# kakao/buffalo

Hardware: NVIDIA H100
Metric: interactions/sec (nnz/s) ALS d=128 (higher is better)
Workload: dtype f32

## Files before the change

buffalo_b200/csrc/als_tc.cuh:

```cuda
#pragma once
#include "als_generic.cuh"
#include "bfl_common.cuh"
#include <type_traits>

#include "sm90_ptx.cuh"

namespace bfl {
namespace tc {

using namespace sm90;

constexpr int N_CONV = 4, KH = N_CONV / 4;
constexpr int W_EPI = 0, W_MMA = 4, W_CONV = 8, W_PLAN = W_CONV + N_CONV;
constexpr int WARPS = 16, THREADS = WARPS * 32;
constexpr int REG_MMA = 200, REG_PLAN = 4 * 128 - 128 - 128 - REG_MMA;
constexpr int NXS = 8;
constexpr int PT = 2;
constexpr int NR = 2;
constexpr int NO = 2;
constexpr int GATHER_AHEAD = 1;
constexpr int NPG = 8, NP = NPG * PT;
constexpr int NBV = 8;
template <int D>
struct Cfg {
    static constexpr int TILE = D == 128 ? 32 : 16;
    static constexpr int NF = D / 128;
    static constexpr int LBO = D * 16;
    static constexpr int OP_BYTES = TILE * D * 2;
};
constexpr uint32_t F_FIRST = 1u << 8, F_LAST = 1u << 9, F_NEG = 1u << 10, F_STOP = 1u << 11;

__device__ __forceinline__ int msw(int c) { return ((c >> 1) & 3) << 3; }

template <int D>
struct Smem {
    static constexpr int TILE = Cfg<D>::TILE;
    alignas(1024) unsigned char op[NO][PT][2][Cfg<D>::OP_BYTES];
    alignas(128) float raw[NR][PT][TILE * D];
    alignas(128) float mat[128 * 128];
    alignas(16) float bvec[NBV][KH][D];
    alignas(16) float sumq[NBV][KH][D];
    alignas(16) float xs[NXS][D];
    alignas(16) float pv[4][32];
    alignas(16) float dl[4][32];
    alignas(16) float sws[NP][TILE];
    alignas(16) float wv[NP][TILE];
    alignas(16) int32_t keys[NP][TILE];
    float wsum[NBV][KH];
    uint32_t meta_raw[NP];
    uint32_t meta_op[NO][PT];
    int badrow[NXS];
    alignas(8) uint64_t plan_full[NPG], plan_empty[NPG], raw_full[NR], raw_empty[NR], op_full[NO], op_empty[NO];
    alignas(8) uint64_t acc_full, acc_empty, x_full[NXS], d_full[4];
};

struct TcArgs {
    AlsArgs a;
    const int32_t* items;
    float* scratch;
    int64_t split;
    int pass;
    int debug;
};

template <int D>
__host__ __device__ constexpr size_t scratch_floats() { return (size_t)D * D + 2 * D + 4; }

__global__ void tc_absmax_kernel(const float* __restrict__ p, size_t n, unsigned int* __restrict__ out) {
    float m = 0.f;
    const size_t gtid = (size_t)blockIdx.x * blockDim.x + threadIdx.x, gsz = (size_t)gridDim.x * blockDim.x;
    const size_t lead = min(n, (size_t)(((16 - ((uintptr_t)p & 15)) & 15) / 4));
    const size_t n4 = (n - lead) / 4;
    const float4* p4 = reinterpret_cast<const float4*>(p + lead);
    for (size_t i = gtid; i < n4; i += gsz) {
        const float4 v = __ldg(p4 + i);
        m = fmaxf(fmaxf(m, fmaxf(fabsf(v.x), fabsf(v.y))), fmaxf(fabsf(v.z), fabsf(v.w)));
    }
    for (size_t i = gtid; i < lead; i += gsz) m = fmaxf(m, fabsf(p[i]));
    for (size_t i = lead + n4 * 4 + gtid; i < n; i += gsz) m = fmaxf(m, fabsf(p[i]));
    for (int o = 16; o > 0; o >>= 1) m = fmaxf(m, __shfl_xor_sync(FULL, m, o));
    if ((threadIdx.x & 31) == 0 && m > 0.f) atomicMax(out, __float_as_uint(m));
}
__global__ void tc_scale_kernel(const unsigned int* __restrict__ ymax, const unsigned int* __restrict__ vmax, float alpha,
                                float* __restrict__ out) {
    const float y = __uint_as_float(*ymax), w = __uint_as_float(*vmax) * fabsf(alpha);
    const float top = y * sqrtf(w);
    int e = 0;
    if (top > 0.f && isfinite(top)) {
        int ex;
        frexpf(top, &ex);
        e = 15 - ex;
    }
    e = max(-60, min(60, e));
    out[0] = ldexpf(1.f, e);
    out[1] = ldexpf(1.f, -2 * e);
}

template <int D, bool PARTIAL, bool LOSS1>
__global__ void __launch_bounds__(THREADS, 1) als_tc_kernel(TcArgs ta) {
    static_assert(D == 128 || (D == 256 && PARTIAL), "fused row solve: d = 128; split-row mode: d = 128 or 256");
    constexpr int TILE = Cfg<D>::TILE, NF = Cfg<D>::NF, LBO = Cfg<D>::LBO;
    extern __shared__ __align__(1024) unsigned char smem_raw_[];
    Smem<D>& S = *reinterpret_cast<Smem<D>*>(smem_raw_);
    const AlsArgs& a = ta.a;
    const int tid = threadIdx.x, lane = tid & 31;
    const int warp = __shfl_sync(FULL, tid >> 5, 0);

    if (tid == 0) {
        for (int i = 0; i < NR; ++i) {
            mbar_init(&S.raw_full[i], N_CONV);
            mbar_init(&S.raw_empty[i], N_CONV);
        }
        for (int i = 0; i < NPG; ++i) {
            mbar_init(&S.plan_full[i], 1);
            mbar_init(&S.plan_empty[i], N_CONV);
        }
        for (int i = 0; i < NO; ++i) {
            mbar_init(&S.op_full[i], N_CONV);
            mbar_init(&S.op_empty[i], 4);
        }
        mbar_init(&S.acc_full, 4);
        mbar_init(&S.acc_empty, 4);
        for (int b = 0; b < 4; ++b) mbar_init(&S.d_full[b], 1);
        for (int i = 0; i < NXS; ++i) {
            mbar_init(&S.x_full[i], 4);
            S.badrow[i] = 0;
        }
        mbar_init_fence();
    }
    __syncthreads();
    const float scale = __ldg(a.tc_scales), inv2 = __ldg(a.tc_scales + 1);

    const int64_t nitems = a.row_end - a.row_begin;
    const int64_t my_first = (int64_t)blockIdx.x;
    const int64_t stride = gridDim.x;

    auto item_info = [&](int64_t it, int& row, int64_t& beg, int64_t& n, int& slot) {
        if (PARTIAL) {
            const int32_t* p = ta.items + 3 * (a.row_begin + it);
            row = p[0];
            const int64_t rb = row == 0 ? 0 : a.indptr[row - 1];
            const int64_t rn = a.indptr[row] - rb;
            beg = rb + (int64_t)p[1] * ta.split;
            n = min(ta.split, rn - (int64_t)p[1] * ta.split);
            slot = p[2];
        } else {
            row = a.row_list[a.row_begin + it];
            beg = row == 0 ? 0 : a.indptr[row - 1];
            n = a.indptr[row] - beg;
            slot = 0;
        }
    };

    if (warp >= W_PLAN) {
        setmaxnreg_dec<REG_PLAN>();
        if (warp != W_PLAN) return;
        uint32_t gsl = 0, rph = 0, pe = 0;
        auto tile_begin = [&]() -> uint32_t {
            if (pe == 0) mbar_wait_idle(&S.plan_empty[gsl], rph ^ 1u);
            return gsl * PT + pe;
        };
        auto tile_end = [&]() {
            if (++pe == PT) {
                if (lane == 0) mbar_arrive(&S.plan_full[gsl]);
                pe = 0;
                if (++gsl == NPG) { gsl = 0; rph ^= 1u; }
            }
        };
        auto emit = [&](unsigned mask, uint32_t flags, int32_t key, float w) {
            const int cnt = __popc(mask);
            const int slot = __popc(mask & ((1u << lane) - 1u));
            const uint32_t rs = tile_begin();
            if ((mask >> lane) & 1u) {
                S.keys[rs][slot] = key;
                S.sws[rs][slot] = sqrtf(fabsf(w)) * scale;
                S.wv[rs][slot] = w;
            } else {
                const int zslot = cnt + lane - slot;
                if (zslot < TILE) {
                    S.sws[rs][zslot] = 0.f;
                    S.wv[rs][zslot] = 0.f;
                }
            }
            if (lane == 0) S.meta_raw[rs] = (uint32_t)cnt | flags;
            __syncwarp();
            tile_end();
        };
        constexpr int SC = 4, SCN = SC * TILE;
        const bool inl = lane < TILE;
        auto load_id = [&](int64_t it, int& row, int& chunk) {
            row = -1;
            chunk = 0;
            if (it < nitems) {
                if (PARTIAL) {
                    const int32_t* p = ta.items + 3 * (a.row_begin + it);
                    row = p[0];
                    chunk = p[1];
                } else {
                    row = a.row_list[a.row_begin + it];
                }
            }
        };
        auto load_span = [&](int row, int chunk, const int32_t*& kp, const float*& vp, int& n) {
            kp = a.keys;
            vp = a.vals;
            n = 0;
            if (row >= 0) {
                const int64_t rb = row == 0 ? 0 : a.indptr[row - 1];
                const int64_t rn = a.indptr[row] - rb;
                int64_t beg = rb;
                n = (int)rn;
                if (PARTIAL) {
                    beg = rb + (int64_t)chunk * ta.split;
                    n = (int)min(ta.split, rn - (int64_t)chunk * ta.split);
                }
                kp = a.keys + (beg - a.shift);
                vp = a.vals + (beg - a.shift);
            }
        };
        auto load_sc = [&](const int32_t* kp, const float* vp, int n, int c0, int32_t (&key)[SC], float (&w)[SC]) {
#pragma unroll
            for (int s = 0; s < SC; ++s) {
                const int idx = c0 + s * TILE + lane;
                const bool ok = inl && idx < n;
                key[s] = ok ? kp[idx] : 0;
                w[s] = ok ? vp[idx] * a.alpha : 0.f;
            }
        };
        auto emit_sc = [&](int n, int c0, const int32_t (&key)[SC], const float (&w)[SC]) {
            bool neg = false;
#pragma unroll
            for (int s = 0; s < SC; ++s) neg |= w[s] < 0.f;
            if (!__any_sync(FULL, neg)) {
#pragma unroll
                for (int s = 0; s < SC; ++s) {
                    const int t0 = c0 + s * TILE;
                    if (t0 < n) {
                        const uint32_t meta = (uint32_t)min(TILE, n - t0) | (t0 == 0 ? F_FIRST : 0u) | (t0 + TILE >= n ? F_LAST : 0u);
                        const uint32_t rs = tile_begin();
                        if (inl) {
                            float sq;
                            asm("sqrt.approx.ftz.f32 %0, %1;" : "=f"(sq) : "f"(w[s]));
                            S.keys[rs][lane] = key[s];
                            S.sws[rs][lane] = sq * scale;
                            S.wv[rs][lane] = w[s];
                        }
                        if (lane == 0) S.meta_raw[rs] = meta;
                        __syncwarp();
                        tile_end();
                    }
                }
            } else {
#pragma unroll
                for (int s = 0; s < SC; ++s) {
                    const int t0 = c0 + s * TILE;
                    if (t0 < n) {
                        const bool valid = inl && t0 + lane < n;
                        const unsigned pm = __ballot_sync(FULL, valid && !(w[s] < 0.f));
                        const unsigned nm = __ballot_sync(FULL, valid && (w[s] < 0.f));
                        const bool lastc = t0 + TILE >= n;
                        uint32_t fl = (t0 == 0 ? F_FIRST : 0u);
                        if (pm) {
                            emit(pm, fl | ((lastc && !nm) ? F_LAST : 0u), key[s], w[s]);
                            fl = 0u;
                        }
                        if (nm) emit(nm, fl | F_NEG | (lastc ? F_LAST : 0u), key[s], w[s]);
                    }
                }
            }
        };
        const int32_t *kp0, *kp1, *kp2, *kp3;
        const float *vp0, *vp1, *vp2, *vp3;
        int n0, n1, n2, n3;
        int row_t, ch_t, row4, ch4;
        int32_t k0[SC], k1[SC], k2[SC], nk[SC];
        float w0[SC], w1[SC], w2[SC], nw[SC];
        load_id(my_first, row_t, ch_t);
        load_span(row_t, ch_t, kp0, vp0, n0);
        load_sc(kp0, vp0, n0, 0, k0, w0);
        load_id(my_first + stride, row_t, ch_t);
        load_span(row_t, ch_t, kp1, vp1, n1);
        load_sc(kp1, vp1, n1, 0, k1, w1);
        load_id(my_first + 2 * stride, row_t, ch_t);
        load_span(row_t, ch_t, kp2, vp2, n2);
        load_id(my_first + 3 * stride, row4, ch4);
        for (int64_t it = my_first; it < nitems; it += stride) {
            load_sc(kp2, vp2, n2, 0, k2, w2);
            load_span(row4, ch4, kp3, vp3, n3);
            load_id(it + 4 * stride, row4, ch4);
            for (int c0 = 0; c0 < n0; c0 += SCN) {
                const bool more = c0 + SCN < n0;
                if (more) load_sc(kp0, vp0, n0, c0 + SCN, nk, nw);
                emit_sc(n0, c0, k0, w0);
                if (more) {
#pragma unroll
                    for (int s = 0; s < SC; ++s) { k0[s] = nk[s]; w0[s] = nw[s]; }
                }
            }
#pragma unroll
            for (int s = 0; s < SC; ++s) { k0[s] = k1[s]; w0[s] = w1[s]; k1[s] = k2[s]; w1[s] = w2[s]; }
            kp0 = kp1; vp0 = vp1; n0 = n1; kp1 = kp2; vp1 = vp2; n1 = n2; kp2 = kp3; vp2 = vp3; n2 = n3;
        }
        do {
            const uint32_t rs = tile_begin();
            if (lane == 0) S.meta_raw[rs] = F_STOP;
            __syncwarp();
            tile_end();
        } while (pe != 0);
    } else if (warp >= W_MMA && warp < W_MMA + 4) {
        setmaxnreg_inc<REG_MMA>();
        const int r0 = (D == 256 && ta.pass == 2) ? 128 : 0, c0 = (D == 256 && ta.pass > 0) ? 128 : 0;
        const int wq = warp - W_MMA;
        const int fr = 16 * wq + (lane >> 2), fc = 2 * (lane & 3);
        float d0[64], d1[64];
        auto acc_init = [&]() {
            const float s2 = scale * scale;
#pragma unroll
            for (int n = 0; n < 16; ++n)
#pragma unroll
                for (int h = 0; h < 2; ++h) {
                    const int r = fr + 8 * h, c = 8 * n + fc;
                    float2 g0 = make_float2(0.f, 0.f), g1 = make_float2(0.f, 0.f);
                    if (!PARTIAL) {
                        g0 = __ldg(reinterpret_cast<const float2*>(a.G + (size_t)r * D + c));
                        g1 = __ldg(reinterpret_cast<const float2*>(a.G + (size_t)(r + 64) * D + c));
                        g0.x += r == c ? a.reg : 0.f;
                        g0.y += r == c + 1 ? a.reg : 0.f;
                        g1.x += r + 64 == c ? a.reg : 0.f;
                        g1.y += r + 64 == c + 1 ? a.reg : 0.f;
                    }
                    d0[4 * n + 2 * h] = g0.x * s2; d0[4 * n + 2 * h + 1] = g0.y * s2;
                    d1[4 * n + 2 * h] = g1.x * s2; d1[4 * n + 2 * h + 1] = g1.y * s2;
                }
        };
        uint32_t os = 0, oph = 0, aph = 0;
        int64_t seq = 0;
        bool stop = false;
        acc_init();
        while (!stop) {
            mbar_wait(&S.op_full[os], oph);
            fence_proxy_async_smem();
#pragma unroll 1
            for (int e = 0; e < PT; ++e) {
                const uint32_t meta = S.meta_op[os][e];
                if (meta & F_STOP) {
                    stop = true;
                    break;
                }
                const int ksteps = (ta.debug & 2) ? 0 : (int)(meta & 0xffu);
                const uint32_t hi = s32(&S.op[os][e][0][0]), lo = s32(&S.op[os][e][1][0]);
                wgmma_fence();
#pragma unroll 1
                for (int ks = 0; ks < ksteps; ++ks) {
                    const uint32_t k0 = ks * 2 * LBO;
                    const uint64_t ah0 = smem_desc(hi + k0 + r0 * 16, LBO, 128), ah1 = smem_desc(hi + k0 + (r0 + 64) * 16, LBO, 128);
                    const uint64_t al0 = smem_desc(lo + k0 + r0 * 16, LBO, 128), al1 = smem_desc(lo + k0 + (r0 + 64) * 16, LBO, 128);
                    const uint64_t bh = smem_desc(hi + k0 + c0 * 16, LBO, 128), bl = smem_desc(lo + k0 + c0 * 16, LBO, 128);
                    if (meta & F_NEG) {
                        wgmma_m64n128k16_f16<true>(d0, ah0, bh);
                        wgmma_m64n128k16_f16<true>(d0, ah0, bl);
                        wgmma_m64n128k16_f16<true>(d0, al0, bh);
                        wgmma_m64n128k16_f16<true>(d1, ah1, bh);
                        wgmma_m64n128k16_f16<true>(d1, ah1, bl);
                        wgmma_m64n128k16_f16<true>(d1, al1, bh);
                    } else {
                        wgmma_m64n128k16_f16<false>(d0, ah0, bh);
                        wgmma_m64n128k16_f16<false>(d0, ah0, bl);
                        wgmma_m64n128k16_f16<false>(d0, al0, bh);
                        wgmma_m64n128k16_f16<false>(d1, ah1, bh);
                        wgmma_m64n128k16_f16<false>(d1, ah1, bl);
                        wgmma_m64n128k16_f16<false>(d1, al1, bh);
                    }
                }
                wgmma_commit();
                if (meta & F_LAST) {
                    wgmma_wait<0>();
#pragma unroll
                    for (int i = 0; i < 64; ++i) { acc_fence(d0[i]); acc_fence(d1[i]); }
                    mbar_wait_idle(&S.acc_empty, aph ^ 1u);
                    if (PARTIAL) {
                        const int slot = ta.items[3 * (a.row_begin + my_first + seq * stride) + 2];
                        float* sc = ta.scratch + (size_t)slot * scratch_floats<D>();
#pragma unroll
                        for (int n = 0; n < 16; ++n)
#pragma unroll
                            for (int h = 0; h < 2; ++h)
#pragma unroll
                                for (int i = 0; i < 2; ++i) {
                                    const int r = r0 + fr + 8 * h, c = c0 + 8 * n + fc + i;
                                    const float v0 = d0[4 * n + 2 * h + i] * inv2, v1 = d1[4 * n + 2 * h + i] * inv2;
                                    atomicAdd(sc + (size_t)r * D + c, v0);
                                    atomicAdd(sc + (size_t)(r + 64) * D + c, v1);
                                    if (r0 != c0) {
                                        atomicAdd(sc + (size_t)c * D + r, v0);
                                        atomicAdd(sc + (size_t)c * D + r + 64, v1);
                                    }
                                }
                    } else {
#pragma unroll
                        for (int n = 0; n < 16; ++n)
#pragma unroll
                            for (int h = 0; h < 2; ++h)
#pragma unroll
                                for (int i = 0; i < 2; ++i) {
                                    const int r = fr + 8 * h, c = 8 * n + fc + i;
                                    S.mat[c * 128 + (r ^ msw(c))] = d0[4 * n + 2 * h + i] * inv2;
                                    S.mat[c * 128 + ((r + 64) ^ msw(c))] = d1[4 * n + 2 * h + i] * inv2;
                                }
                    }
                    __syncwarp();
                    if (lane == 0) mbar_arrive(&S.acc_full);
                    aph ^= 1u;
                    ++seq;
                    acc_init();
                }
            }
            wgmma_wait<0>();
#pragma unroll
            for (int i = 0; i < 64; ++i) { acc_fence(d0[i]); acc_fence(d1[i]); }
            __syncwarp();
            if (lane == 0) mbar_arrive(&S.op_empty[os]);
            if (++os == NO) { os = 0; oph ^= 1u; }
        }
    } else if (warp >= W_CONV && warp < W_CONV + N_CONV) {
        const int cta = tid - W_CONV * 32;
        const int ct = cta & 127;
        const int kh = cta >> 7;
        constexpr int CHS = TILE / 8 / KH;
        uint32_t rs = 0, rph = 0, os = 0, oph = 0, bslot = 0;
        float2 bacc[NF], qacc[NF];
        float wacc = 0.f;
#pragma unroll
        for (int f = 0; f < NF; ++f) { bacc[f] = make_float2(0.f, 0.f); qacc[f] = make_float2(0.f, 0.f); }
        const int cw = cta >> 5;
        uint32_t gs = 0, gph = 0, grs = 0, grph = 0;
        bool plan_end = false;
        auto gather = [&]() {
            if (plan_end) {
                cp_async_commit();
                return;
            }
            mbar_wait(&S.plan_full[gs], gph);
            mbar_wait(&S.raw_empty[grs], grph ^ 1u);
            const uint32_t gm0 = S.meta_raw[gs * PT], gm1 = S.meta_raw[gs * PT + 1];
            if (PT == 2 && !(ta.debug & 1) && ((gm0 | gm1) & F_STOP) == 0 && (gm0 & 0xffu) == TILE && (gm1 & 0xffu) == TILE) {
                int32_t kk[PT][TILE / N_CONV];
#pragma unroll
                for (int e = 0; e < PT; ++e)
#pragma unroll
                    for (int i = 0; i < TILE / N_CONV; ++i) kk[e][i] = S.keys[gs * PT + e][cw + N_CONV * i];
#pragma unroll
                for (int e = 0; e < PT; ++e)
#pragma unroll
                    for (int i = 0; i < TILE / N_CONV; ++i) {
                        const float* src = a.Y + (int64_t)kk[e][i] * a.ld + lane * 4;
                        float* dst = &S.raw[grs][e][(cw + N_CONV * i) * D + lane * 4];
#pragma unroll
                        for (int c = 0; c < D / 128; ++c) cp_async16_cg(dst + c * 128, src + c * 128);
                    }
            } else
#pragma unroll
            for (int e = 0; e < PT; ++e) {
                const uint32_t gmeta = S.meta_raw[gs * PT + e];
                if (gmeta & F_STOP) {
                    plan_end = true;
                } else {
                    const int gcnt = (ta.debug & 1) ? 0 : (int)(gmeta & 0xffu);
#pragma unroll
                    for (int i = 0; i < TILE / N_CONV; ++i) {
                        const int slot = cw + N_CONV * i;
                        if (slot < gcnt) {
                            const float* src = a.Y + (int64_t)S.keys[gs * PT + e][slot] * a.ld + lane * 4;
                            float* dst = &S.raw[grs][e][slot * D + lane * 4];
#pragma unroll
                            for (int c = 0; c < D / 128; ++c) cp_async16_cg(dst + c * 128, src + c * 128);
                        }
                    }
                }
            }
            cp_async_commit();
            if (++gs == NPG) { gs = 0; gph ^= 1u; }
            if (++grs == NR) { grs = 0; grph ^= 1u; }
        };
        uint32_t cs = 0;
        bool done = false;
        if (ta.debug & 16) {
            uint32_t ph = 0;
            for (;;) {
                mbar_wait(&S.plan_full[cs], ph);
                const bool stop = (S.meta_raw[cs * PT] | S.meta_raw[cs * PT + 1]) & F_STOP;
                __syncwarp();
                if (lane == 0) mbar_arrive(&S.plan_empty[cs]);
                if (stop) break;
                if (++cs == NPG) { cs = 0; ph ^= 1u; }
            }
            if (cta == 0) S.meta_op[0][0] = F_STOP;
            __syncwarp();
            if (lane == 0) mbar_arrive(&S.op_full[0]);
            done = true;
        }
#pragma unroll 1
        for (int i = 0; i < GATHER_AHEAD && !done; ++i) gather();
        while (!done) {
            gather();
            cp_async_wait_group<GATHER_AHEAD>();
            __syncwarp();
            if (lane == 0) mbar_arrive(&S.raw_full[rs]);
            mbar_wait(&S.raw_full[rs], rph);
            float qv[PT][CHS * 8 * NF];
#pragma unroll
            for (int e = 0; e < PT; ++e)
#pragma unroll
                for (int c = 0; c < CHS; ++c)
#pragma unroll
                    for (int i = 0; i < 8; ++i)
#pragma unroll
                        for (int f = 0; f < NF; ++f)
                            qv[e][(c * 8 + i) * NF + f] = S.raw[rs][e][((kh * CHS + c) * 8 + i) * D + ct + 128 * f];
            mbar_wait(&S.op_empty[os], oph ^ 1u);
            const uint32_t cm0 = S.meta_raw[cs * PT], cm1 = S.meta_raw[cs * PT + 1];
            const bool fast2 = PT == 2 && !(ta.debug & 4) && ((cm0 | cm1) & F_STOP) == 0 && (cm0 & 0xffu) == TILE &&
                               (cm1 & 0xffu) == TILE;
            if (fast2) {
#pragma unroll
                for (int e = 0; e < PT; ++e) {
                    const uint32_t meta = e == 0 ? cm0 : cm1;
                    const uint32_t psl = cs * PT + e;
                    const bool first = (meta & F_FIRST) != 0;
#pragma unroll
                    for (int f = 0; f < NF; ++f) {
                        bacc[f].x = first ? 0.f : bacc[f].x; bacc[f].y = first ? 0.f : bacc[f].y;
                        qacc[f].x = first ? 0.f : qacc[f].x; qacc[f].y = first ? 0.f : qacc[f].y;
                    }
                    wacc = first ? 0.f : wacc;
                    unsigned char* hi = &S.op[os][e][0][0];
                    unsigned char* lo = &S.op[os][e][1][0];
#pragma unroll
                    for (int c = 0; c < CHS; ++c) {
                        const int kc = kh * CHS + c, k0 = kc * 8;
                        const float4 sa = *reinterpret_cast<const float4*>(&S.sws[psl][k0]);
                        const float4 sb = *reinterpret_cast<const float4*>(&S.sws[psl][k0 + 4]);
                        const float4 wa = *reinterpret_cast<const float4*>(&S.wv[psl][k0]);
                        const float4 wb = *reinterpret_cast<const float4*>(&S.wv[psl][k0 + 4]);
                        if (LOSS1) wacc += ((wa.x + wa.y) + (wa.z + wa.w)) + ((wb.x + wb.y) + (wb.z + wb.w));
#pragma unroll
                        for (int f = 0; f < NF; ++f) {
                            const int m = ct + 128 * f;
                            const float* q = &qv[e][0];
                            const float2 q01 = make_float2(q[(c * 8 + 0) * NF + f], q[(c * 8 + 1) * NF + f]);
                            const float2 q23 = make_float2(q[(c * 8 + 2) * NF + f], q[(c * 8 + 3) * NF + f]);
                            const float2 q45 = make_float2(q[(c * 8 + 4) * NF + f], q[(c * 8 + 5) * NF + f]);
                            const float2 q67 = make_float2(q[(c * 8 + 6) * NF + f], q[(c * 8 + 7) * NF + f]);
                            uint4 h4, l4;
                            split_f16x2(f2mul(q01, make_float2(sa.x, sa.y)), h4.x, l4.x);
                            split_f16x2(f2mul(q23, make_float2(sa.z, sa.w)), h4.y, l4.y);
                            split_f16x2(f2mul(q45, make_float2(sb.x, sb.y)), h4.z, l4.z);
                            split_f16x2(f2mul(q67, make_float2(sb.z, sb.w)), h4.w, l4.w);
                            const int off = kc * LBO + (m >> 3) * 128 + (m & 7) * 16;
                            *reinterpret_cast<uint4*>(hi + off) = h4;
                            *reinterpret_cast<uint4*>(lo + off) = l4;
                            bacc[f] = f2fma(make_float2(wa.x, wa.y), q01, bacc[f]);
                            bacc[f] = f2fma(make_float2(wa.z, wa.w), q23, bacc[f]);
                            bacc[f] = f2fma(make_float2(wb.x, wb.y), q45, bacc[f]);
                            bacc[f] = f2fma(make_float2(wb.z, wb.w), q67, bacc[f]);
                            if (LOSS1) {
                                qacc[f].x += (q01.x + q23.x) + (q45.x + q67.x);
                                qacc[f].y += (q01.y + q23.y) + (q45.y + q67.y);
                            }
                        }
                    }
#pragma unroll
                    for (int f = 0; f < NF; ++f) {
                        S.bvec[bslot][kh][ct + 128 * f] = bacc[f].x + bacc[f].y;
                        if (LOSS1) S.sumq[bslot][kh][ct + 128 * f] = qacc[f].x + qacc[f].y;
                    }
                    if (LOSS1 && ct == 0) S.wsum[bslot][kh] = wacc;
                    bslot = (bslot + ((meta & F_LAST) ? 1u : 0u)) & (NBV - 1);
                    if (cta == 0) S.meta_op[os][e] = (uint32_t)(TILE / 16) | (meta & (F_FIRST | F_LAST | F_NEG));
                }
            } else
#pragma unroll
            for (int e = 0; e < PT; ++e) {
                if (done) continue;
                const uint32_t psl = cs * PT + e;
                const uint32_t meta = S.meta_raw[psl];
                if (meta & F_STOP) {
                    if (cta == 0) S.meta_op[os][e] = F_STOP;
                    done = true;
                    continue;
                }
                const int cnt = (int)(meta & 0xffu), ksteps = (cnt + 15) >> 4;
                if (meta & F_FIRST) {
#pragma unroll
                    for (int f = 0; f < NF; ++f) { bacc[f] = make_float2(0.f, 0.f); qacc[f] = make_float2(0.f, 0.f); }
                    wacc = 0.f;
                }
                unsigned char* hi = &S.op[os][e][0][0];
                unsigned char* lo = &S.op[os][e][1][0];
                auto chunk = [&](auto guard, const int c) {
                    constexpr bool GUARD = decltype(guard)::value;
                    const int kc = kh * CHS + c, k0 = kc * 8;
                    const float4 sa = *reinterpret_cast<const float4*>(&S.sws[psl][k0]);
                    const float4 sb = *reinterpret_cast<const float4*>(&S.sws[psl][k0 + 4]);
                    const float4 wa = *reinterpret_cast<const float4*>(&S.wv[psl][k0]);
                    const float4 wb = *reinterpret_cast<const float4*>(&S.wv[psl][k0 + 4]);
                    if (LOSS1) wacc += ((wa.x + wa.y) + (wa.z + wa.w)) + ((wb.x + wb.y) + (wb.z + wb.w));
#pragma unroll
                    for (int f = 0; f < NF; ++f) {
                        const int m = ct + 128 * f;
                        float q[8];
#pragma unroll
                        for (int i = 0; i < 8; ++i) q[i] = qv[e][(c * 8 + i) * NF + f];
                        if (GUARD) {
#pragma unroll
                            for (int i = 0; i < 8; ++i) q[i] = (k0 + i < cnt) ? q[i] : 0.f;
                        }
                        const float2 q01 = make_float2(q[0], q[1]), q23 = make_float2(q[2], q[3]);
                        const float2 q45 = make_float2(q[4], q[5]), q67 = make_float2(q[6], q[7]);
                        uint4 h4, l4;
                        split_f16x2(f2mul(q01, make_float2(sa.x, sa.y)), h4.x, l4.x);
                        split_f16x2(f2mul(q23, make_float2(sa.z, sa.w)), h4.y, l4.y);
                        split_f16x2(f2mul(q45, make_float2(sb.x, sb.y)), h4.z, l4.z);
                        split_f16x2(f2mul(q67, make_float2(sb.z, sb.w)), h4.w, l4.w);
                        const int off = kc * LBO + (m >> 3) * 128 + (m & 7) * 16;
                        *reinterpret_cast<uint4*>(hi + off) = h4;
                        *reinterpret_cast<uint4*>(lo + off) = l4;
                        bacc[f] = f2fma(make_float2(wa.x, wa.y), q01, bacc[f]);
                        bacc[f] = f2fma(make_float2(wa.z, wa.w), q23, bacc[f]);
                        bacc[f] = f2fma(make_float2(wb.x, wb.y), q45, bacc[f]);
                        bacc[f] = f2fma(make_float2(wb.z, wb.w), q67, bacc[f]);
                        if (LOSS1) {
                            qacc[f].x += (q[0] + q[2]) + (q[4] + q[6]);
                            qacc[f].y += (q[1] + q[3]) + (q[5] + q[7]);
                        }
                    }
                };
                if (ta.debug & 4) {
                } else if (cnt == TILE) {
#pragma unroll
                    for (int c = 0; c < CHS; ++c) chunk(std::false_type{}, c);
                } else {
#pragma unroll
                    for (int c = 0; c < CHS; ++c)
                        if (kh * CHS + c < 2 * ksteps) chunk(std::true_type{}, c);
                }
                if (meta & F_LAST) {
#pragma unroll
                    for (int f = 0; f < NF; ++f) {
                        S.bvec[bslot][kh][ct + 128 * f] = bacc[f].x + bacc[f].y;
                        if (LOSS1) S.sumq[bslot][kh][ct + 128 * f] = qacc[f].x + qacc[f].y;
                    }
                    if (LOSS1 && ct == 0) S.wsum[bslot][kh] = wacc;
                    bslot = (bslot + 1) & (NBV - 1);
                }
                if (cta == 0) S.meta_op[os][e] = (uint32_t)ksteps | (meta & (F_FIRST | F_LAST | F_NEG));
            }
            __syncwarp();
            if (lane == 0) {
                mbar_arrive(&S.raw_empty[rs]);
                mbar_arrive(&S.plan_empty[cs]);
                mbar_arrive(&S.op_full[os]);
            }
            cs = (cs + 1) & (NPG - 1);
            if (++rs == NR) { rs = 0; rph ^= 1u; }
            if (++os == NO) { os = 0; oph ^= 1u; }
        }
    } else {
        const int q = warp & 3;
        const int j = q * 32 + lane;
        float* pv = S.pv[q];
        double l_nume = 0.0, l_deno = 0.0;
        const float tol = a.tol;
        if constexpr (PARTIAL) {
            int row = 0, slot = 0, nrow = 0, nslot = 0;
            int64_t beg, n = 0, nbeg, nn = 0;
            if (my_first < nitems) item_info(my_first, row, beg, n, slot);
            for (int64_t seq = 0; my_first + seq * stride < nitems; ++seq) {
                const int64_t nit = my_first + (seq + 1) * stride;
                if (nit < nitems) item_info(nit, nrow, nbeg, nn, nslot);
                const uint32_t aph = (uint32_t)(seq & 1);
                const uint32_t bs = (uint32_t)(seq & (NBV - 1));
                mbar_wait_idle(&S.acc_full, aph);
                float* sc = ta.scratch + (size_t)slot * scratch_floats<D>();
                if (ta.pass == 0) {
                    for (int jj = j; jj < D; jj += 128) {
                        atomicAdd(sc + (size_t)D * D + jj, S.bvec[bs][0][jj] + (KH == 2 ? S.bvec[bs][KH - 1][jj] : 0.f));
                        if (LOSS1) atomicAdd(sc + (size_t)D * D + D + jj, S.sumq[bs][0][jj] + (KH == 2 ? S.sumq[bs][KH - 1][jj] : 0.f));
                    }
                    if (LOSS1 && j == 0) atomicAdd(sc + (size_t)D * D + 2 * D, S.wsum[bs][0] + (KH == 2 ? S.wsum[bs][KH - 1] : 0.f));
                }
                __syncwarp();
                if (lane == 0) mbar_arrive(&S.acc_empty);
                row = nrow; slot = nslot; n = nn;
            }
        } else {
            auto row_of = [&](int64_t sq) -> int {
                const int64_t it = my_first + sq * stride;
                return it < nitems ? a.row_list[a.row_begin + it] : -1;
            };
            auto len_of = [&](int row) -> float {
                if (row < 0 || !a.compute_loss) return 0.f;
                return (float)(a.indptr[row] - (row == 0 ? 0 : a.indptr[row - 1]));
            };
            int row = (ta.debug & 16) ? -1 : row_of(0), row1 = row_of(1), row2 = row_of(2);
            float xj = row >= 0 ? a.X[(int64_t)row * a.ld + j] : 0.f;
            float x1 = row1 >= 0 ? a.X[(int64_t)row1 * a.ld + j] : 0.f;
            float nlen = len_of(row), nlen1 = len_of(row1);
            if (row >= 0) {
                S.xs[0][j] = xj;
                __syncwarp();
                if (lane == 0) mbar_arrive(&S.x_full[0]);
            }
            auto mat = [&](int c) -> float { return S.mat[c * 128 + (j ^ msw(c))]; };
            for (int64_t seq = 0; row >= 0; ++seq) {
                const int row3 = row_of(seq + 3);
                const float x2 = row2 >= 0 ? a.X[(int64_t)row2 * a.ld + j] : 0.f;
                const float nlen2 = len_of(row2);
                if (row1 >= 0) {
                    S.xs[(seq + 1) & (NXS - 1)][j] = x1;
                    __syncwarp();
                    if (lane == 0) mbar_arrive(&S.x_full[(seq + 1) & (NXS - 1)]);
                }
                const uint32_t aph = (uint32_t)(seq & 1);
                const uint32_t bs = (uint32_t)(seq & (NBV - 1));
                const uint32_t xsl = (uint32_t)(seq & (NXS - 1));
                const float* xs = S.xs[xsl];
                mbar_wait(&S.x_full[xsl], (uint32_t)((seq / NXS) & 1));
                mbar_wait_idle(&S.acc_full, aph);
                if (ta.debug & 8) {
                    __syncwarp();
                    if (lane == 0) mbar_arrive(&S.acc_empty);
                    row = row1; row1 = row2; row2 = row3;
                    xj = x1; x1 = x2;
                    continue;
                }
                const float bj = S.bvec[bs][0][j] + (KH == 2 ? S.bvec[bs][KH - 1][j] : 0.f);
                float hM = 0.f;
                float md[32];
#pragma unroll
                for (int c = 0; c < D / 32; ++c) {
                    float h0 = 0.f, h1 = 0.f;
#pragma unroll
                    for (int i = 0; i < 32; i += 4) {
                        const float4 x4 = *reinterpret_cast<const float4*>(xs + c * 32 + i);
                        const float m0 = mat(c * 32 + i), m1 = mat(c * 32 + i + 1), m2 = mat(c * 32 + i + 2), m3 = mat(c * 32 + i + 3);
                        h0 = fmaf(m0, x4.x, h0); h1 = fmaf(m1, x4.y, h1);
                        h0 = fmaf(m2, x4.z, h0); h1 = fmaf(m3, x4.w, h1);
                        if (c == q) { md[i] = m0; md[i + 1] = m1; md[i + 2] = m2; md[i + 3] = m3; }
                    }
                    hM += h0 + h1;
                }
                if (a.compute_loss) {
                    const float kappa = a.adaptive_reg ? nlen : 1.0f;
                    double t = (double)(kappa * a.reg * xj * xj);
                    if (a.axis == 1) {
                        t += (double)xj * (double)hM - (double)(a.reg * xj * xj) -
                             2.0 * (double)xj * ((double)bj + (double)S.sumq[bs][0][j] + (KH == 2 ? (double)S.sumq[bs][KH - 1][j] : 0.0));
                        if (j == 0) {
                            const double ws = (double)S.wsum[bs][0] + (KH == 2 ? (double)S.wsum[bs][KH - 1] : 0.0);
                            t += (double)nlen + ws;
                            l_deno += (double)a.Y_rows + ws;
                        }
                    }
                    l_nume += t;
                }
                float h = hM - bj;
#pragma unroll 1
                for (int B = 0; B < q; ++B) {
                    float mv[32];
#pragma unroll
                    for (int i = 0; i < 32; ++i) mv[i] = mat(B * 32 + i);
                    mbar_wait(&S.d_full[B], aph);
                    float u0 = 0.f, u1 = 0.f;
#pragma unroll
                    for (int i = 0; i < 32; i += 4) {
                        const float4 d4 = *reinterpret_cast<const float4*>(&S.dl[B][i]);
                        u0 = fmaf(mv[i], d4.x, u0);
                        u1 = fmaf(mv[i + 1], d4.y, u1);
                        u0 = fmaf(mv[i + 2], d4.z, u0);
                        u1 = fmaf(mv[i + 3], d4.w, u1);
                    }
                    h -= u0 + u1;
                }
                __syncwarp();
                if (lane == 0) mbar_arrive(&S.acc_empty);
                float xv = 0.f;
                {
                    float r = h, p = h;
                    float rsold = warp_sum(r * r);
                    bool act = rsold > tol;
#pragma unroll 1
                    for (int step = 0; step < 3; ++step) {
                        pv[lane] = p;
                        __syncwarp();
                        float a0 = 0.f, a1 = 0.f, a2 = 0.f, a3 = 0.f;
#pragma unroll
                        for (int i = 0; i < 32; i += 4) {
                            const float4 p4 = *reinterpret_cast<const float4*>(pv + i);
                            a0 = fmaf(md[i], p4.x, a0); a1 = fmaf(md[i + 1], p4.y, a1);
                            a2 = fmaf(md[i + 2], p4.z, a2); a3 = fmaf(md[i + 3], p4.w, a3);
                        }
                        __syncwarp();
                        const float Ap = (a0 + a1) + (a2 + a3);
                        const float pAp = warp_sum(p * Ap);
                        const float ss = act ? __fdividef(rsold, pAp) : 0.f;
                        xv = fmaf(ss, p, xv);
                        r = fmaf(-ss, Ap, r);
                        const float rsnew = warp_sum(r * r);
                        act = act && !(rsnew < tol);
                        if (act) p = fmaf(__fdividef(rsnew, rsold), p, r);
                        rsold = act ? rsnew : rsold;
                    }
                }
                float v = xj - xv;
                const bool badw = __any_sync(FULL, !isfinite(v));
                a.X[(int64_t)row * a.ld + j] = v;
                for (int pr = 0; pr < a.n_peer; ++pr) a.peerX[pr][(int64_t)row * a.ld + j] = v;
                if (q < 3) {
                    S.dl[q][lane] = xv;
                    if (badw && lane == 0) atomicOr(&S.badrow[xsl], 1);
                    __syncwarp();
                    if (lane == 0) mbar_arrive(&S.d_full[q]);
                }
                if (q == 3) {
                    const bool bad = badw || (S.badrow[xsl] != 0);
                    if (bad) {
#pragma unroll
                        for (int c = 0; c < 4; ++c) {
                            a.X[(int64_t)row * a.ld + c * 32 + lane] = 0.f;
                            for (int pr = 0; pr < a.n_peer; ++pr) a.peerX[pr][(int64_t)row * a.ld + c * 32 + lane] = 0.f;
                        }
                        __syncwarp();
                        if (lane == 0) S.badrow[xsl] = 0;
                    }
                }
                row = row1; row1 = row2; row2 = row3;
                xj = x1; x1 = x2;
                nlen = nlen1; nlen1 = nlen2;
            }
            if (a.loss && a.compute_loss) {
                l_nume = warp_sum_d(l_nume);
                l_deno = warp_sum_d(l_deno);
                if (lane == 0 && (l_nume != 0.0 || l_deno != 0.0)) {
                    atomicAdd(a.loss, l_nume);
                    atomicAdd(a.loss + 1, l_deno);
                }
            }
        }
    }
}

inline bool tc_applicable(int optimizer_code, int d, int vdim, int block_size) {
    return optimizer_code == 8 && d == 128 && vdim == 128 && block_size == 32;
}
inline bool tc_split_applicable(int optimizer_code, int d, int vdim, int block_size) {
    return optimizer_code == 8 && (d == 128 || d == 256) && vdim == d && block_size == 32;
}

inline int tc_note_absmax(const float* p, size_t n, unsigned int* out, int num_sms, cudaStream_t st) {
    BFL_CUDA(cudaMemsetAsync(out, 0, sizeof(unsigned int), st));
    if (n == 0) return BFL_OK;
    const int grid = (int)std::min<size_t>((n / 4 + 255) / 256 + 1, (size_t)num_sms * 8);
    tc_absmax_kernel<<<grid, 256, 0, st>>>(p, n, out);
    BFL_LAUNCHED();
    return BFL_OK;
}
inline int tc_update_scale(const unsigned int* ymax, const unsigned int* vmax, float alpha, float* scales, cudaStream_t st) {
    tc_scale_kernel<<<1, 1, 0, st>>>(ymax, vmax, alpha, scales);
    BFL_LAUNCHED();
    return BFL_OK;
}

__global__ void tc_count_items_kernel(const int64_t* __restrict__ indptr, const int32_t* __restrict__ list, int64_t nrows,
                                      int64_t split, unsigned long long* total) {
    for (int64_t i = (int64_t)blockIdx.x * blockDim.x + threadIdx.x; i < nrows; i += (int64_t)gridDim.x * blockDim.x) {
        const int row = list[i];
        const int64_t n = indptr[row] - (row == 0 ? 0 : indptr[row - 1]);
        atomicAdd(total, (unsigned long long)((n + split - 1) / split));
    }
}
__global__ void tc_fill_items_kernel(const int64_t* __restrict__ indptr, const int32_t* __restrict__ list, int64_t nrows,
                                     int64_t split, unsigned long long* cursor, int32_t* __restrict__ items) {
    for (int64_t i = (int64_t)blockIdx.x * blockDim.x + threadIdx.x; i < nrows; i += (int64_t)gridDim.x * blockDim.x) {
        const int row = list[i];
        const int64_t n = indptr[row] - (row == 0 ? 0 : indptr[row - 1]);
        const int64_t nc = (n + split - 1) / split;
        const unsigned long long pos = atomicAdd(cursor, (unsigned long long)nc);
        for (int64_t c = 0; c < nc; ++c) {
            items[3 * (pos + c) + 0] = row;
            items[3 * (pos + c) + 1] = (int32_t)c;
            items[3 * (pos + c) + 2] = (int32_t)i;
        }
    }
}

template <int D>
int tc_launch_partial(const AlsArgs& a, const int32_t* items, int64_t nitems, float* scratch, int64_t nslots,
                      int64_t split, int num_sms, cudaStream_t st) {
    if (nitems <= 0) return BFL_OK;
    if (!a.tc_scales) BFL_FAIL(BFL_ERR_STATE, "tensor-core ALS kernel: operand scale not prepared");
    TcArgs ta;
    ta.a = a;
    ta.a.row_begin = 0;
    ta.a.row_end = nitems;
    ta.items = items;
    ta.scratch = scratch;
    ta.split = split;
    ta.debug = 0;
    BFL_CUDA(cudaMemsetAsync(scratch, 0, sizeof(float) * scratch_floats<D>() * (size_t)nslots, st));
    const size_t smem = sizeof(Smem<D>);
    const int grid = (int)std::min<int64_t>(nitems, (int64_t)num_sms);
    for (ta.pass = 0; ta.pass < (D == 128 ? 1 : 3); ++ta.pass) {
        if (a.compute_loss && a.axis == 1) {
            BFL_CUDA(cudaFuncSetAttribute(als_tc_kernel<D, true, true>, cudaFuncAttributeMaxDynamicSharedMemorySize, (int)smem));
            als_tc_kernel<D, true, true><<<grid, THREADS, smem, st>>>(ta);
        } else {
            BFL_CUDA(cudaFuncSetAttribute(als_tc_kernel<D, true, false>, cudaFuncAttributeMaxDynamicSharedMemorySize, (int)smem));
            als_tc_kernel<D, true, false><<<grid, THREADS, smem, st>>>(ta);
        }
        BFL_LAUNCHED();
    }
    return BFL_OK;
}

inline int tc_launch(const AlsArgs& a, int num_sms, cudaStream_t st) {
    const int64_t nrows = a.row_end - a.row_begin;
    if (nrows <= 0) return BFL_OK;
    if (!a.tc_scales) BFL_FAIL(BFL_ERR_STATE, "tensor-core ALS kernel: operand scale not prepared");
    TcArgs ta;
    ta.a = a;
    ta.items = nullptr;
    ta.scratch = nullptr;
    ta.split = 0;
    ta.pass = 0;
    ta.debug = getenv("BFL_TC_DEBUG") ? atoi(getenv("BFL_TC_DEBUG")) : 0;
    const size_t smem = sizeof(Smem<128>);
    const int grid = (int)std::min<int64_t>(nrows, (int64_t)num_sms);
    if (a.compute_loss && a.axis == 1) {
        BFL_CUDA(cudaFuncSetAttribute(als_tc_kernel<128, false, true>, cudaFuncAttributeMaxDynamicSharedMemorySize, (int)smem));
        als_tc_kernel<128, false, true><<<grid, THREADS, smem, st>>>(ta);
    } else {
        BFL_CUDA(cudaFuncSetAttribute(als_tc_kernel<128, false, false>, cudaFuncAttributeMaxDynamicSharedMemorySize, (int)smem));
        als_tc_kernel<128, false, false><<<grid, THREADS, smem, st>>>(ta);
    }
    BFL_LAUNCHED();
    return BFL_OK;
}

}
}
```

buffalo_b200/csrc/sm90_ptx.cuh:

```cuda
#pragma once
#include <cuda_runtime.h>
#include <stdint.h>

namespace bfl {
namespace sm90 {

__device__ __forceinline__ uint32_t s32(const void* p) { return (uint32_t)__cvta_generic_to_shared(p); }

__device__ __forceinline__ void mbar_init(uint64_t* bar, uint32_t count) {
    asm volatile("mbarrier.init.shared::cta.b64 [%0], %1;" ::"r"(s32(bar)), "r"(count) : "memory");
}
__device__ __forceinline__ void mbar_init_fence() { asm volatile("fence.mbarrier_init.release.cluster;" ::: "memory"); }
__device__ __forceinline__ void mbar_arrive(uint64_t* bar) {
    asm volatile("mbarrier.arrive.shared::cta.b64 _, [%0];" ::"r"(s32(bar)) : "memory");
}
__device__ __forceinline__ bool mbar_try_wait(uint64_t* bar, uint32_t parity) {
    uint32_t ok;
    asm volatile(
        "{\n\t.reg .pred p;\n\t"
        "mbarrier.try_wait.parity.shared::cta.b64 p, [%1], %2;\n\t"
        "selp.b32 %0, 1, 0, p;\n\t}"
        : "=r"(ok)
        : "r"(s32(bar)), "r"(parity)
        : "memory");
    return ok != 0;
}
__device__ __forceinline__ void mbar_wait(uint64_t* bar, uint32_t parity) {
    while (!mbar_try_wait(bar, parity)) {
    }
}
__device__ __forceinline__ void mbar_wait_idle(uint64_t* bar, uint32_t parity) {
    while (!mbar_try_wait(bar, parity)) __nanosleep(128);
}

__device__ __forceinline__ void fence_proxy_async_smem() { asm volatile("fence.proxy.async.shared::cta;" ::: "memory"); }

__device__ __forceinline__ void cp_async16_cg(void* smem_dst, const void* gsrc) {
    asm volatile("cp.async.cg.shared.global [%0], [%1], 16;" ::"r"(s32(smem_dst)), "l"(gsrc) : "memory");
}
__device__ __forceinline__ void cp_async_commit() { asm volatile("cp.async.commit_group;" ::: "memory"); }
template <int N>
__device__ __forceinline__ void cp_async_wait_group() { asm volatile("cp.async.wait_group %0;" ::"n"(N) : "memory"); }

__device__ __forceinline__ uint64_t smem_desc(uint32_t saddr, uint32_t lbo_bytes, uint32_t sbo_bytes) {
    return (uint64_t)((saddr >> 4) & 0x3fffu) | ((uint64_t)((lbo_bytes >> 4) & 0x3fffu) << 16) |
           ((uint64_t)((sbo_bytes >> 4) & 0x3fffu) << 32);
}
__device__ __forceinline__ void wgmma_fence() { asm volatile("wgmma.fence.sync.aligned;" ::: "memory"); }
__device__ __forceinline__ void wgmma_commit() { asm volatile("wgmma.commit_group.sync.aligned;" ::: "memory"); }
template <int N>
__device__ __forceinline__ void wgmma_wait() { asm volatile("wgmma.wait_group.sync.aligned %0;" ::"n"(N) : "memory"); }
template <int N>
__device__ __forceinline__ void setmaxnreg_inc() { asm volatile("setmaxnreg.inc.sync.aligned.u32 %0;" ::"n"(N)); }
template <int N>
__device__ __forceinline__ void setmaxnreg_dec() { asm volatile("setmaxnreg.dec.sync.aligned.u32 %0;" ::"n"(N)); }
__device__ __forceinline__ void acc_fence(float& r) { asm volatile("" : "+f"(r)::"memory"); }

#define BFL_WGMMA_ACC64(d)                                                                                              \
    "+f"(d[0]), "+f"(d[1]), "+f"(d[2]), "+f"(d[3]), "+f"(d[4]), "+f"(d[5]), "+f"(d[6]), "+f"(d[7]), "+f"(d[8]),         \
        "+f"(d[9]), "+f"(d[10]), "+f"(d[11]), "+f"(d[12]), "+f"(d[13]), "+f"(d[14]), "+f"(d[15]), "+f"(d[16]),        \
        "+f"(d[17]), "+f"(d[18]), "+f"(d[19]), "+f"(d[20]), "+f"(d[21]), "+f"(d[22]), "+f"(d[23]), "+f"(d[24]),       \
        "+f"(d[25]), "+f"(d[26]), "+f"(d[27]), "+f"(d[28]), "+f"(d[29]), "+f"(d[30]), "+f"(d[31]), "+f"(d[32]),       \
        "+f"(d[33]), "+f"(d[34]), "+f"(d[35]), "+f"(d[36]), "+f"(d[37]), "+f"(d[38]), "+f"(d[39]), "+f"(d[40]),       \
        "+f"(d[41]), "+f"(d[42]), "+f"(d[43]), "+f"(d[44]), "+f"(d[45]), "+f"(d[46]), "+f"(d[47]), "+f"(d[48]),       \
        "+f"(d[49]), "+f"(d[50]), "+f"(d[51]), "+f"(d[52]), "+f"(d[53]), "+f"(d[54]), "+f"(d[55]), "+f"(d[56]),       \
        "+f"(d[57]), "+f"(d[58]), "+f"(d[59]), "+f"(d[60]), "+f"(d[61]), "+f"(d[62]), "+f"(d[63])
#define BFL_WGMMA_REGS64                                                                                                \
    "{%0, %1, %2, %3, %4, %5, %6, %7, %8, %9, %10, %11, %12, %13, %14, %15, %16, %17, %18, %19, %20, %21, %22, %23, "   \
    "%24, %25, %26, %27, %28, %29, %30, %31, %32, %33, %34, %35, %36, %37, %38, %39, %40, %41, %42, %43, %44, %45, %46, " \
    "%47, %48, %49, %50, %51, %52, %53, %54, %55, %56, %57, %58, %59, %60, %61, %62, %63}"
template <bool NEG>
__device__ __forceinline__ void wgmma_m64n128k16_f16(float (&d)[64], uint64_t adesc, uint64_t bdesc) {
    if (NEG) {
        asm volatile("wgmma.mma_async.sync.aligned.m64n128k16.f32.f16.f16 " BFL_WGMMA_REGS64 ", %64, %65, 1, -1, 1, 0, 0;"
                     : BFL_WGMMA_ACC64(d)
                     : "l"(adesc), "l"(bdesc)
                     : "memory");
    } else {
        asm volatile("wgmma.mma_async.sync.aligned.m64n128k16.f32.f16.f16 " BFL_WGMMA_REGS64 ", %64, %65, 1, 1, 1, 0, 0;"
                     : BFL_WGMMA_ACC64(d)
                     : "l"(adesc), "l"(bdesc)
                     : "memory");
    }
}
#undef BFL_WGMMA_ACC64
#undef BFL_WGMMA_REGS64

__device__ __forceinline__ float2 f2mul(float2 a, float2 b) { return make_float2(__fmul_rn(a.x, b.x), __fmul_rn(a.y, b.y)); }
__device__ __forceinline__ float2 f2fma(float2 a, float2 b, float2 c) {
    return make_float2(fmaf(a.x, b.x, c.x), fmaf(a.y, b.y, c.y));
}
__device__ __forceinline__ void split_f16x2(float2 s, uint32_t& head, uint32_t& tail) {
    float2 h;
    h.x = __uint_as_float(__float_as_uint(s.x) & 0xffffe000u);
    h.y = __uint_as_float(__float_as_uint(s.y) & 0xffffe000u);
    const float2 t = f2fma(h, make_float2(-1.f, -1.f), s);
    asm("cvt.rn.f16x2.f32 %0, %1, %2;" : "=r"(head) : "f"(h.y), "f"(h.x));
    asm("cvt.rn.f16x2.f32 %0, %1, %2;" : "=r"(tail) : "f"(t.y), "f"(t.x));
}

}
}
```

Measured before the change: 1.015 billion.

## Exploit Gram symmetry: compute only lower-triangular blocks of the 128x128 accumulator

For the non-partial path, the 128x128 Gram accumulator is symmetric. The upper-left 64x128 block now uses an m64n64 WGMMA (columns 0-63 only), and the missing upper-right 64x64 block is filled in by mirroring the lower-left block from d1 during the epilogue store. This cuts tensor-core work per k-step by about a quarter and frees 32 accumulator registers per thread. In exchange it adds extra shared-memory stores in the epilogue and relies on the operands being symmetric (A equals B).

```diff
diff --git a/buffalo_b200/csrc/als_tc.cuh b/buffalo_b200/csrc/als_tc.cuh
--- a/buffalo_b200/csrc/als_tc.cuh
+++ b/buffalo_b200/csrc/als_tc.cuh
@@ -312,7 +312,9 @@
         const int r0 = (D == 256 && ta.pass == 2) ? 128 : 0, c0 = (D == 256 && ta.pass > 0) ? 128 : 0;
         const int wq = warp - W_MMA;
         const int fr = 16 * wq + (lane >> 2), fc = 2 * (lane & 3);
-        float d0[64], d1[64];
+        constexpr bool SYM = !PARTIAL;
+        constexpr int N0 = SYM ? 8 : 16;
+        float d0[4 * N0], d1[64];
         auto acc_init = [&]() {
             const float s2 = scale * scale;
 #pragma unroll
@@ -322,16 +324,22 @@
                     const int r = fr + 8 * h, c = 8 * n + fc;
                     float2 g0 = make_float2(0.f, 0.f), g1 = make_float2(0.f, 0.f);
                     if (!PARTIAL) {
-                        g0 = __ldg(reinterpret_cast<const float2*>(a.G + (size_t)r * D + c));
+                        if (n < N0) g0 = __ldg(reinterpret_cast<const float2*>(a.G + (size_t)r * D + c));
                         g1 = __ldg(reinterpret_cast<const float2*>(a.G + (size_t)(r + 64) * D + c));
                         g0.x += r == c ? a.reg : 0.f;
                         g0.y += r == c + 1 ? a.reg : 0.f;
                         g1.x += r + 64 == c ? a.reg : 0.f;
                         g1.y += r + 64 == c + 1 ? a.reg : 0.f;
                     }
-                    d0[4 * n + 2 * h] = g0.x * s2; d0[4 * n + 2 * h + 1] = g0.y * s2;
+                    if (n < N0) { d0[4 * n + 2 * h] = g0.x * s2; d0[4 * n + 2 * h + 1] = g0.y * s2; }
                     d1[4 * n + 2 * h] = g1.x * s2; d1[4 * n + 2 * h + 1] = g1.y * s2;
                 }
+        };
+        auto acc_fence_all = [&]() {
+#pragma unroll
+            for (int i = 0; i < 4 * N0; ++i) acc_fence(d0[i]);
+#pragma unroll
+            for (int i = 0; i < 64; ++i) acc_fence(d1[i]);
         };
         uint32_t os = 0, oph = 0, aph = 0;
         int64_t seq = 0;
@@ -356,17 +364,32 @@
                     const uint64_t ah0 = smem_desc(hi + k0 + r0 * 16, LBO, 128), ah1 = smem_desc(hi + k0 + (r0 + 64) * 16, LBO, 128);
                     const uint64_t al0 = smem_desc(lo + k0 + r0 * 16, LBO, 128), al1 = smem_desc(lo + k0 + (r0 + 64) * 16, LBO, 128);
                     const uint64_t bh = smem_desc(hi + k0 + c0 * 16, LBO, 128), bl = smem_desc(lo + k0 + c0 * 16, LBO, 128);
+                    if constexpr (SYM) {
+                        if (meta & F_NEG) {
+                            wgmma_m64n64k16_f16<true>(d0, ah0, bh);
+                            wgmma_m64n64k16_f16<true>(d0, ah0, bl);
+                            wgmma_m64n64k16_f16<true>(d0, al0, bh);
+                        } else {
+                            wgmma_m64n64k16_f16<false>(d0, ah0, bh);
+                            wgmma_m64n64k16_f16<false>(d0, ah0, bl);
+                            wgmma_m64n64k16_f16<false>(d0, al0, bh);
+                        }
+                    } else {
+                        if (meta & F_NEG) {
+                            wgmma_m64n128k16_f16<true>(d0, ah0, bh);
+                            wgmma_m64n128k16_f16<true>(d0, ah0, bl);
+                            wgmma_m64n128k16_f16<true>(d0, al0, bh);
+                        } else {
+                            wgmma_m64n128k16_f16<false>(d0, ah0, bh);
+                            wgmma_m64n128k16_f16<false>(d0, ah0, bl);
+                            wgmma_m64n128k16_f16<false>(d0, al0, bh);
+                        }
+                    }
                     if (meta & F_NEG) {
-                        wgmma_m64n128k16_f16<true>(d0, ah0, bh);
-                        wgmma_m64n128k16_f16<true>(d0, ah0, bl);
-                        wgmma_m64n128k16_f16<true>(d0, al0, bh);
                         wgmma_m64n128k16_f16<true>(d1, ah1, bh);
                         wgmma_m64n128k16_f16<true>(d1, ah1, bl);
                         wgmma_m64n128k16_f16<true>(d1, al1, bh);
                     } else {
-                        wgmma_m64n128k16_f16<false>(d0, ah0, bh);
-                        wgmma_m64n128k16_f16<false>(d0, ah0, bl);
-                        wgmma_m64n128k16_f16<false>(d0, al0, bh);
                         wgmma_m64n128k16_f16<false>(d1, ah1, bh);
                         wgmma_m64n128k16_f16<false>(d1, ah1, bl);
                         wgmma_m64n128k16_f16<false>(d1, al1, bh);
@@ -375,10 +398,9 @@
                 wgmma_commit();
                 if (meta & F_LAST) {
                     wgmma_wait<0>();
-#pragma unroll
-                    for (int i = 0; i < 64; ++i) { acc_fence(d0[i]); acc_fence(d1[i]); }
+                    acc_fence_all();
                     mbar_wait_idle(&S.acc_empty, aph ^ 1u);
-                    if (PARTIAL) {
+                    if constexpr (PARTIAL) {
                         const int slot = ta.items[3 * (a.row_begin + my_first + seq * stride) + 2];
                         float* sc = ta.scratch + (size_t)slot * scratch_floats<D>();
 #pragma unroll
@@ -404,8 +426,12 @@
 #pragma unroll
                                 for (int i = 0; i < 2; ++i) {
                                     const int r = fr + 8 * h, c = 8 * n + fc + i;
-                                    S.mat[c * 128 + (r ^ msw(c))] = d0[4 * n + 2 * h + i] * inv2;
-                                    S.mat[c * 128 + ((r + 64) ^ msw(c))] = d1[4 * n + 2 * h + i] * inv2;
+                                    const float v1 = d1[4 * n + 2 * h + i] * inv2;
+                                    if (n < N0) {
+                                        S.mat[c * 128 + (r ^ msw(c))] = d0[4 * n + 2 * h + i] * inv2;
+                                        S.mat[(r + 64) * 128 + (c ^ msw(r))] = v1;
+                                    }
+                                    S.mat[c * 128 + ((r + 64) ^ msw(c))] = v1;
                                 }
                     }
                     __syncwarp();
@@ -416,8 +442,7 @@
                 }
             }
             wgmma_wait<0>();
-#pragma unroll
-            for (int i = 0; i < 64; ++i) { acc_fence(d0[i]); acc_fence(d1[i]); }
+            acc_fence_all();
             __syncwarp();
             if (lane == 0) mbar_arrive(&S.op_empty[os]);
             if (++os == NO) { os = 0; oph ^= 1u; }
diff --git a/buffalo_b200/csrc/sm90_ptx.cuh b/buffalo_b200/csrc/sm90_ptx.cuh
--- a/buffalo_b200/csrc/sm90_ptx.cuh
+++ b/buffalo_b200/csrc/sm90_ptx.cuh
@@ -86,6 +86,31 @@
 #undef BFL_WGMMA_ACC64
 #undef BFL_WGMMA_REGS64
 
+#define BFL_WGMMA_ACC32(d)                                                                                              \
+    "+f"(d[0]), "+f"(d[1]), "+f"(d[2]), "+f"(d[3]), "+f"(d[4]), "+f"(d[5]), "+f"(d[6]), "+f"(d[7]), "+f"(d[8]),         \
+        "+f"(d[9]), "+f"(d[10]), "+f"(d[11]), "+f"(d[12]), "+f"(d[13]), "+f"(d[14]), "+f"(d[15]), "+f"(d[16]),        \
+        "+f"(d[17]), "+f"(d[18]), "+f"(d[19]), "+f"(d[20]), "+f"(d[21]), "+f"(d[22]), "+f"(d[23]), "+f"(d[24]),       \
+        "+f"(d[25]), "+f"(d[26]), "+f"(d[27]), "+f"(d[28]), "+f"(d[29]), "+f"(d[30]), "+f"(d[31])
+#define BFL_WGMMA_REGS32                                                                                                \
+    "{%0, %1, %2, %3, %4, %5, %6, %7, %8, %9, %10, %11, %12, %13, %14, %15, %16, %17, %18, %19, %20, %21, %22, %23, "   \
+    "%24, %25, %26, %27, %28, %29, %30, %31}"
+template <bool NEG>
+__device__ __forceinline__ void wgmma_m64n64k16_f16(float (&d)[32], uint64_t adesc, uint64_t bdesc) {
+    if (NEG) {
+        asm volatile("wgmma.mma_async.sync.aligned.m64n64k16.f32.f16.f16 " BFL_WGMMA_REGS32 ", %32, %33, 1, -1, 1, 0, 0;"
+                     : BFL_WGMMA_ACC32(d)
+                     : "l"(adesc), "l"(bdesc)
+                     : "memory");
+    } else {
+        asm volatile("wgmma.mma_async.sync.aligned.m64n64k16.f32.f16.f16 " BFL_WGMMA_REGS32 ", %32, %33, 1, 1, 1, 0, 0;"
+                     : BFL_WGMMA_ACC32(d)
+                     : "l"(adesc), "l"(bdesc)
+                     : "memory");
+    }
+}
+#undef BFL_WGMMA_ACC32
+#undef BFL_WGMMA_REGS32
+
 __device__ __forceinline__ float2 f2mul(float2 a, float2 b) { return make_float2(__fmul_rn(a.x, b.x), __fmul_rn(a.y, b.y)); }
 __device__ __forceinline__ float2 f2fma(float2 a, float2 b, float2 c) {
     return make_float2(fmaf(a.x, b.x, c.x), fmaf(a.y, b.y, c.y));
```

Result: faster. 1.096 billion (median of 6 runs) (+8.0%).
